# uthree/tinyvc

Measured on AMD Instinct MI355X. Metric: audio-samples/sec (16 kHz) end-to-end VC, higher is better.
Workload: dtype f32 (fp32 in / out / accumulate; channel contractions as two-term fp16 splits on v_mfma_f32_32x32x16_f16: 22-bit significands, three part-products per fp32 product)

## Files before the change

### tinyvc_amd/csrc/encoder.hip

```cpp
#include "conv3s.h"
#include "gemm_s2.h"
#include "cnx_s3.h"
#include "small_kernels.h"
#include "tvc_common.h"

namespace tvc {

constexpr int ENC_MTB = 4, ENC_NWV = 4, ENC_BPC = 2;

template <bool DW, int CPT>
static __global__ __launch_bounds__(1024) void dwconv_ln_kernel(const float* x, float* y,
                                                               const float* __restrict__ dw_w, const float* __restrict__ dw_b,
                                                               const float* __restrict__ g, const float* __restrict__ bta,
                                                               int C, int T, int dil, RagDev rg) {
    constexpr int NW = 16;
    const int rs = T;
    long ubase = (long)blockIdx.y * C * T;
    if (rg.tb) {
        T = rg.tb[blockIdx.y];
        ubase = rg.pre[blockIdx.y];
        if ((int)blockIdx.x * 64 >= T) return;
    }
    __shared__ float red[NW][64];
    constexpr bool STAGE = CPT >= 16;
    __shared__ __attribute__((aligned(16))) float Wl[STAGE ? 16 * CPT * 8 : 8];
    __shared__ float Gl[2][STAGE ? 16 * CPT : 1];
    if (STAGE) {
        for (int i = threadIdx.x; i < C; i += 1024) {
            if (DW) {
#pragma unroll
                for (int j = 0; j < 7; ++j) Wl[i * 8 + j] = dw_w[i * 7 + j];
                Wl[i * 8 + 7] = dw_b[i];
            }
            Gl[0][i] = g[i];
            Gl[1][i] = bta[i];
        }
        __syncthreads();
    }
    const int lane = threadIdx.x & 63, wave = threadIdx.x >> 6;
    const int t = blockIdx.x * 64 + lane;
    const bool ok = t < T;
    const int tc = ok ? t : T - 1;
    const float* xb = x + ubase;
    float* yb = y + ubase;

    int tt[7];
#pragma unroll
    for (int j = 0; j < 7; ++j) {
        int q = tc + (j - 3) * dil;
        tt[j] = q < 0 ? 0 : (q >= T ? T - 1 : q);
    }
    float v[CPT];
    float sum = 0.f;
#pragma unroll
    for (int i = 0; i < CPT; ++i) {
        const int c = wave + i * NW;
        if (DW) {
            const float* xr = xb + (long)c * rs;
            float wj[7], a;
            if (STAGE) {
                const float4 w0 = *reinterpret_cast<const float4*>(Wl + c * 8), w1 = *reinterpret_cast<const float4*>(Wl + c * 8 + 4);
                wj[0] = w0.x; wj[1] = w0.y; wj[2] = w0.z; wj[3] = w0.w; wj[4] = w1.x; wj[5] = w1.y; wj[6] = w1.z;
                a = w1.w;
            } else {
#pragma unroll
                for (int j = 0; j < 7; ++j) wj[j] = dw_w[c * 7 + j];
                a = dw_b[c];
            }
#pragma unroll
            for (int j = 0; j < 7; ++j) a = fmaf(wj[j], xr[tt[j]], a);
            v[i] = a;
        } else {
            v[i] = xb[(long)c * rs + tc];
        }
        sum += v[i];
    }
    red[wave][lane] = sum;
    __syncthreads();
    float tot = 0.f;
#pragma unroll
    for (int w = 0; w < NW; ++w) tot += red[w][lane];
    const float mean = tot / (float)C;
    __syncthreads();
    float sq = 0.f;
#pragma unroll
    for (int i = 0; i < CPT; ++i) {
        const float d = v[i] - mean;
        sq = fmaf(d, d, sq);
    }
    red[wave][lane] = sq;
    __syncthreads();
    float tot2 = 0.f;
#pragma unroll
    for (int w = 0; w < NW; ++w) tot2 += red[w][lane];
    const float var = tot2 / (float)C;
    const float rstd = 1.f / sqrtf(var + 1e-5f);
    if (!ok) return;
#pragma unroll
    for (int i = 0; i < CPT; ++i) {
        const int c = wave + i * NW;
        yb[(long)c * rs + t] = fmaf((v[i] - mean) * rstd, STAGE ? Gl[0][c] : g[c], STAGE ? Gl[1][c] : bta[c]);
    }
}
template <bool DW>
static int dwconv_ln_launch(tvc_ctx* ctx, hipStream_t s, const float* x, float* y, const float* dw_w, const float* dw_b, const float* g,
                            const float* bta, int B, int C, int T, int dil) {
    RagDev rg;
    TVC_CHECK(rag_view(ctx, s, 1, 0, &rg, nullptr));
    const dim3 grid(((ctx->rag ? ctx->rag->Tlong : T) + 63) / 64, ctx->rag ? ctx->rag->B : B), blk(1024);
    if (C == 384) hipLaunchKernelGGL((dwconv_ln_kernel<DW, 24>), grid, blk, 0, s, x, y, dw_w, dw_b, g, bta, C, T, dil, rg);
    else if (C == 128) hipLaunchKernelGGL((dwconv_ln_kernel<DW, 8>), grid, blk, 0, s, x, y, dw_w, dw_b, g, bta, C, T, dil, rg);
    else return fail(ctx, TVC_ERR_ARG, "dwconv_ln: unsupported channel count %d", C);
    return 0;
}

static __global__ void grn_norm_kernel(const float* __restrict__ h, float* __restrict__ gx, long rows, int T, RagDev rg, int C2) {
    const int lane = threadIdx.x & 63;
    long wave = (blockIdx.x * (long)blockDim.x + threadIdx.x) >> 6;
    long nwaves = ((long)gridDim.x * blockDim.x) >> 6;
    for (long r = wave; r < rows; r += nwaves) {
        const float* p = h + r * T;
        int n = T;
        if (rg.tb) {
            const int b = (int)(r / C2), c = (int)(r - (long)b * C2);
            p = h + (long)c * T + rg.pre[b];
            n = rg.tb[b];
        }
        float s = 0.f;
        for (int t = lane; t < n; t += 64) s = fmaf(p[t], p[t], s);
#pragma unroll
        for (int o = 32; o > 0; o >>= 1) s += __shfl_xor(s, o);
        if (lane == 0) gx[r] = sqrtf(s);
    }
}

static __global__ __launch_bounds__(256) void grn_finalize_kernel(const float* __restrict__ gx, const float* __restrict__ gamma,
                                                                  float* __restrict__ nx, int C2, float* __restrict__ hmax) {
    __shared__ float red[4];
    __shared__ float redm[4];
    const int b = blockIdx.x;
    const float* g = gx + (long)b * C2;
    float s = 0.f;
    for (int c = threadIdx.x; c < C2; c += 256) s += g[c];
#pragma unroll
    for (int o = 32; o > 0; o >>= 1) s += __shfl_xor(s, o);
    if ((threadIdx.x & 63) == 0) red[threadIdx.x >> 6] = s;
    __syncthreads();
    const float mean = (red[0] + red[1] + red[2] + red[3]) / (float)C2;
    const float den = mean + 1e-6f;
    float mx = 0.f;
    for (int c = threadIdx.x; c < C2; c += 256) {
        const float f = fmaf(gamma[c], g[c] / den, 1.f);
        nx[(long)b * C2 + c] = f;
        mx = fmaxf(mx, g[c] * fabsf(f));
    }
#pragma unroll
    for (int o = 32; o > 0; o >>= 1) mx = fmaxf(mx, __shfl_xor(mx, o));
    if ((threadIdx.x & 63) == 0) redm[threadIdx.x >> 6] = mx;
    __syncthreads();
    if (threadIdx.x == 0) hmax[b] = fmaxf(fmaxf(redm[0], redm[1]), fmaxf(redm[2], redm[3]));
}

int run_layernorm(tvc_ctx* ctx, hipStream_t s, float* x, const float* g, const float* b, int B, int C, int T) {
    TVC_CHECK(dwconv_ln_launch<false>(ctx, s, x, x, nullptr, nullptr, g, b, B, C, T, 1));
    return launch_check(ctx, "layernorm");
}

static __global__ void grn_tiles_kernel(float* __restrict__ gp, int gp_tiles, int K, int T, RagDev rg) {
    const int b = blockIdx.y, c = blockIdx.x * blockDim.x + threadIdx.x;
    if (c >= K) return;
    const int Tb = rg.tb ? rg.tb[b] : T, n = (Tb + 63) / 64;
    float* g = gp + (long)b * gp_tiles * K + c;
    float s = g[0];
    for (int t = 1; t < n; ++t) s += g[(long)t * K];
    g[0] = s;
}

template <int C>
static bool cnx_try(int* rc, tvc_ctx* ctx, hipStream_t s, const ConvNeXtW& w, float* x, float* h, float* gx, int B, int T, float* amax_out) {
    if (w.C != C || !(w.ln_bound < 32768.f) || w.c2.MT6 != 2 * C / 32 || w.c3.MT6 != C / 32 || w.c2.S6 < C / 16 || w.c3.S6 < 2 * C / 16) return false;
    const int NB = ctx->rag ? ctx->rag->B : B, Tl = ctx->rag ? ctx->rag->Tlong : T, rs = T;
    if ((long)rs * 8 * 4 >= (1L << 31)) return false;
    constexpr int KP = C == 384 ? 2 : 1;
    if ((*rc = lds_optin<cnx1_kernel<C, 1>>(ctx, Cnx1<C, 1>::LDS_BYTES, "cnx")) ||
        (*rc = lds_optin<cnx1_kernel<C, 2>>(ctx, Cnx1<C, 2>::LDS_BYTES, "cnx")) ||
        (*rc = lds_optin<cnx2_kernel<C, KP>>(ctx, Cnx2<C, KP>::LDS_BYTES, "cnx")))
        return true;
    CnxArgs a{};
    a.x = x;
    a.h = h;
    a.T = T;
    a.rs = rs;
    if ((*rc = rag_view(ctx, s, 1, 0, &a.rg, nullptr)) != 0) return true;
    auto split = [&](int MT, int tiles) {
        int d = 1;
        for (int c = 1; c <= MT; ++c)
            if (MT % c == 0 && (long)tiles * c <= ctx->ncu) d = c;
        return d;
    };
    {
        a.A6 = reinterpret_cast<const uint4*>(w.c2.A6);
        a.wsc = w.c2.wscale;
        a.bias = w.c2.bias;
        a.MT = w.c2.MT6;
        a.dw_w = w.dw_w;
        a.dw_b = w.dw_b;
        a.ln_g = w.ln_g;
        a.ln_b = w.ln_b;
        a.dil = w.dilation;
        const int nt = Tl <= 32 ? 1 : 2, tx = (Tl + 32 * nt - 1) / (32 * nt);
        a.gp = gx;
        a.gp_tiles = tx;
        const int d = split(a.MT, tx * NB);
        a.mt_per_wg = a.MT / d;
        const dim3 grid((unsigned)tx, (unsigned)NB, (unsigned)d);
        constexpr int nthr = Cnx1<C, 2>::NTHR, lds1 = Cnx1<C, 1>::LDS_BYTES, lds2 = Cnx1<C, 2>::LDS_BYTES;
        if (nt == 1) hipLaunchKernelGGL((cnx1_kernel<C, 1>), grid, dim3(nthr), lds1, s, a);
        else hipLaunchKernelGGL((cnx1_kernel<C, 2>), grid, dim3(nthr), lds2, s, a);
    }
    a.gp_sum = a.gp_tiles > CNX_GP_INLINE;
    if (a.gp_sum) hipLaunchKernelGGL(grn_tiles_kernel, dim3((2 * C + 255) / 256, (unsigned)NB), dim3(256), 0, s, gx, a.gp_tiles, 2 * C, T, a.rg);
    {
        a.A6 = reinterpret_cast<const uint4*>(w.c3.A6);
        a.wsc = w.c3.wscale;
        a.bias = w.c3_bias_grn;
        a.MT = w.c3.MT6;
        a.grn_g = w.grn_g;
        a.amax_y = amax_out;
        const int tx = (Tl + 63) / 64;
        const int d = split(a.MT, tx * NB);
        a.mt_per_wg = a.MT / d;
        constexpr int nthr = Cnx2<C, KP>::NTHR, lds = Cnx2<C, KP>::LDS_BYTES;
        hipLaunchKernelGGL((cnx2_kernel<C, KP>), dim3((unsigned)tx, (unsigned)NB, (unsigned)d), dim3(nthr), lds, s, a);
    }
    *rc = launch_check(ctx, "convnext (fused)");
    return true;
}

int run_convnext(tvc_ctx* ctx, hipStream_t s, Ws& ws, const ConvNeXtW& w, float* x, int B, int T, float* amax_out) {
    const int C = w.C, C2 = 2 * w.C, ncols = B * T;
    const int NB = ctx->rag ? ctx->rag->B : B;
    size_t mk = ws.mark();
    float* y = ws.get<float>((size_t)B * C * T);
    float* h = ws.get<float>((size_t)B * C2 * T);
    const int Tlong = ctx->rag ? ctx->rag->Tlong : T;
    float* gx = ws.get<float>((size_t)NB * C2 * ((Tlong + 63) / 64));
    float* nx = ws.get<float>((size_t)NB * C2);
    float* ymax = ws.get<float>((size_t)NB);
    float* hmax = ws.get<float>((size_t)NB);
    ws.release(mk);
    if (ws.dry) return 0;
    {
        int rc = 0;
        if (C == 384 ? cnx_try<384>(&rc, ctx, s, w, x, h, gx, B, T, amax_out) : (C == 128 && cnx_try<128>(&rc, ctx, s, w, x, h, gx, B, T, amax_out))) return rc;
    }
    {
        TVC_CHECK(dwconv_ln_launch<true>(ctx, s, x, y, w.dw_w, w.dw_b, w.ln_g, w.ln_b, B, C, T, w.dilation));
    }
    {
        const float* ym = nullptr;
        if (!(w.ln_bound < 32768.f)) {
            TVC_HIP(ctx, hipMemsetAsync(ymax, 0, (size_t)NB * sizeof(float), s));
            TVC_CHECK(run_amax_rows(ctx, s, y, B, C, T, ymax));
            ym = ymax;
        }
        EpiBias<ACT_GELU, false> ep{h, w.c2.bias, nullptr, C2, T, ncols, (long)C2 * T, 0};
        int rc = 0;
        if (!gemm_s2_try(&rc, ctx, s, w.c2, y, B, C, T, 0, ep, ym)) rc = gemm_s_launch<ENC_MTB, ENC_NWV, ENC_BPC>(ctx, s, w.c2, y, B, C, T, 0, ep, ym);
        TVC_CHECK(rc);
    }
    {
        RagDev rg;
        TVC_CHECK(rag_view(ctx, s, 1, 0, &rg, nullptr));
        hipLaunchKernelGGL(grn_norm_kernel, dim3(grid_for((long)NB * C2 * 64)), dim3(256), 0, s, h, gx, (long)NB * C2, T, rg, C2);
        hipLaunchKernelGGL(grn_finalize_kernel, dim3(NB), dim3(256), 0, s, gx, w.grn_g, nx, C2, hmax);
    }
    {
        EpiBias<ACT_NONE, true> ep{x, w.c3_bias_grn, x, C, T, ncols, (long)C * T, (long)C * T};
        int rc = 0;
        if (!gemm_s2_try<EpiBias<ACT_NONE, true>, true>(&rc, ctx, s, w.c3, h, B, C2, T, 0, ep, hmax, nx))
            rc = gemm_s_launch<ENC_MTB, ENC_NWV, ENC_BPC, EpiBias<ACT_NONE, true>, true>(ctx, s, w.c3, h, B, C2, T, 0, ep, hmax, nx);
        TVC_CHECK(rc);
    }
    if (amax_out) TVC_CHECK(run_amax_rows(ctx, s, x, B, C, T, amax_out));
    return launch_check(ctx, "convnext");
}

struct EpiSplit {
    static constexpr bool kIgemm = true;
    float* y0;
    float* y1;
    const float* bias;
    int M0, M1, T, ncols;
    __device__ __forceinline__ void store(int n, int m, const float v[4]) const {
        if (n >= ncols) return;
        int b = n / T, t = n - b * T;
#pragma unroll
        for (int r = 0; r < 4; ++r) {
            int mm = m + r;
            float o = v[r] + bias[mm < M0 + M1 ? mm : 0];
            if (mm < M0)
                y0[((long)b * M0 + mm) * T + t] = o;
            else if (mm < M0 + M1)
                y1[((long)b * M1 + mm - M0) * T + t] = o;
        }
    }
};

struct PTop4 {
    float v[4];
    int i[4];
    __device__ __forceinline__ void init() {
#pragma unroll
        for (int j = 0; j < 4; ++j) { v[j] = -INFINITY; i[j] = 0x7fffffff; }
    }
    __device__ __forceinline__ static bool better(float a, int ia, float b, int ib) { return a > b || (a == b && ia < ib); }
    __device__ __forceinline__ void insert(float x, int ix) {
        if (!better(x, ix, v[3], i[3])) return;
        if (better(x, ix, v[0], i[0])) { v[3] = v[2]; i[3] = i[2]; v[2] = v[1]; i[2] = i[1]; v[1] = v[0]; i[1] = i[0]; v[0] = x; i[0] = ix; }
        else if (better(x, ix, v[1], i[1])) { v[3] = v[2]; i[3] = i[2]; v[2] = v[1]; i[2] = i[1]; v[1] = x; i[1] = ix; }
        else if (better(x, ix, v[2], i[2])) { v[3] = v[2]; i[3] = i[2]; v[2] = x; i[2] = ix; }
        else { v[3] = x; i[3] = ix; }
    }
};

constexpr int kPdWaves = 16;
static __global__ __launch_bounds__(kPdWaves * 64) void pitch_decode_kernel(const float* __restrict__ logits, const float* __restrict__ freq,
                                                                  float* __restrict__ f0, int B, int T, float* __restrict__ f0s, float shift,
                                                                  const float* __restrict__ shifts, const int* __restrict__ col2b) {
    __shared__ float sv[kPdWaves][4][64];
    __shared__ int si[kPdWaves][4][64];
    const int lane = threadIdx.x & 63, wave = threadIdx.x >> 6;
    const long ncols = (long)B * T;
    const long n = blockIdx.x * 64L + lane;
    const bool ok = n < ncols;
    const long nn = ok ? n : ncols - 1;
    const int b = (int)(nn / T), t = (int)(nn - (long)b * T);
    const float* p = logits + (long)b * kPitchClasses * T + t;
    PTop4 top;
    top.init();
    constexpr int CPW = kPitchClasses / kPdWaves;
    float xv[CPW];
#pragma unroll
    for (int j = 0; j < CPW; ++j) xv[j] = p[(long)(wave * CPW + j) * T];
#pragma unroll
    for (int j = 0; j < CPW; ++j) {
        const float x = xv[j];
        top.insert(x != x ? INFINITY : x, wave * CPW + j);
    }
#pragma unroll
    for (int e = 0; e < 4; ++e) { sv[wave][e][lane] = top.v[e]; si[wave][e][lane] = top.i[e]; }
    __syncthreads();
    if (wave != 0 || !ok) return;
    for (int w = 1; w < kPdWaves; ++w)
#pragma unroll
        for (int e = 0; e < 4; ++e) top.insert(sv[w][e][lane], si[w][e][lane]);
#pragma unroll
    for (int e = 0; e < 4; ++e) top.i[e] = (unsigned)top.i[e] < (unsigned)kPitchClasses ? top.i[e] : 0;
    const float v0 = top.v[0];
    float e0 = 1.f, e1 = (float)exp((double)(top.v[1] - v0)), e2 = (float)exp((double)(top.v[2] - v0)), e3 = (float)exp((double)(top.v[3] - v0));
    float den = ((e0 + e1) + e2) + e3;
    float acc = __fmul_rn(e0 / den, freq[top.i[0]]);
    acc = __fadd_rn(acc, __fmul_rn(e1 / den, freq[top.i[1]]));
    acc = __fadd_rn(acc, __fmul_rn(e2 / den, freq[top.i[2]]));
    acc = __fadd_rn(acc, __fmul_rn(e3 / den, freq[top.i[3]]));
    const float fv = acc <= 20.f ? 0.f : acc;
    f0[n] = fv;
    if (f0s) f0s[n] = shift_frequency_one(fv, shifts ? shifts[col2b ? col2b[n] : b] : shift);
}

int run_pitch_decode(tvc_ctx* ctx, hipStream_t s, const float* logits, float* f0, int B, int T) {
    if (!ctx->pitch_freq) return fail(ctx, TVC_ERR_STATE, "pitch table not uploaded (tvc_set_pitch_table + tvc_finalize_weights)");
    const long ncols = (long)B * T;
    hipLaunchKernelGGL(pitch_decode_kernel, dim3((unsigned)((ncols + 63) / 64)), dim3(kPdWaves * 64), 0, s, logits, ctx->pitch_freq, f0, B, T, (float*)nullptr, 0.f, (const float*)nullptr, (const int*)nullptr);
    return launch_check(ctx, "pitch_decode");
}

int run_encoder(tvc_ctx* ctx, hipStream_t s, Ws& ws, const float* spec, float* ssl, float* f0,
                float* logits, int B, int T, const float* spec_bound, float* zeroed_slots, float* f0_shifted, float shift, const float* shifts) {
    const int ncols = B * T;
    float* xs = ws.get<float>((size_t)B * kSslCh * T);
    float* xp = ws.get<float>((size_t)B * kPitchCh * T);
    float* lg = logits ? logits : ws.get<float>((size_t)B * kPitchClasses * T);
    const int NB = ctx->rag ? ctx->rag->B : B;
    float* slots = zeroed_slots ? zeroed_slots : ws.get<float>((size_t)3 * NB);
    float *spec_max = slots, *xs_max = slots + NB, *xp_max = slots + 2 * NB;
    if (!ws.dry) {
        if (!zeroed_slots) TVC_HIP(ctx, hipMemsetAsync(slots, 0, (size_t)3 * NB * sizeof(float), s));
        if (spec_bound) spec_max = const_cast<float*>(spec_bound);
        else TVC_CHECK(run_amax_rows(ctx, s, spec, B, kBins, T, spec_max));
        EpiSplit ep{xs, xp, ctx->enc_in.bias, kSslCh, kPitchCh, T, ncols};
        TVC_CHECK((gemm_s_launch_ragged<ENC_MTB, ENC_NWV, ENC_BPC>(ctx, s, ctx->enc_in, spec, B, kBins, T, (long)kBins * T, ep, spec_max)));
        TVC_CHECK(run_layernorm(ctx, s, xs, ctx->ssl_ln_g, ctx->ssl_ln_b, B, kSslCh, T));
        TVC_CHECK(run_layernorm(ctx, s, xp, ctx->pit_ln_g, ctx->pit_ln_b, B, kPitchCh, T));
    }
    const int gtiles = ((ctx->rag ? ctx->rag->Tlong : T) + 63) / 64;
    const size_t ssl_scratch = ((size_t)B * kSslCh * T * 3 + (size_t)NB * kSslCh * 2 * (gtiles + 1)) * sizeof(float) + (size_t)NB * 8 + 4096;
    char* ssl_blk = ws.get<char>(ssl_scratch);
    Ws wssl(ssl_blk, ssl_scratch, ws.dry);
    SideFork fk(ctx, s);
    TVC_CHECK(fk.fork(ws, ctx->ev_fork, ctx->ev_join));
    const hipStream_t sp = fk.side;
    for (int i = 0; i < 4; ++i) TVC_CHECK(run_convnext(ctx, sp, ws, ctx->pit_mid[i], xp, B, T, i == 3 ? xp_max : nullptr));
    if (!ws.dry) {
        EpiBias<ACT_NONE, false> ep{lg, ctx->pit_out.bias, nullptr, kPitchClasses, T, ncols, (long)kPitchClasses * T, 0};
        int rc = 0;
        if (!gemm_s2_try(&rc, ctx, sp, ctx->pit_out, xp, B, kPitchCh, T, 0, ep, xp_max)) rc = gemm_s_launch<ENC_MTB, ENC_NWV, ENC_BPC>(ctx, sp, ctx->pit_out, xp, B, kPitchCh, T, 0, ep, xp_max);
        TVC_CHECK(rc);
        hipLaunchKernelGGL(pitch_decode_kernel, dim3((ncols + 63) / 64), dim3(kPdWaves * 64), 0, sp, lg, ctx->pitch_freq, f0, B, T, f0_shifted, shift, shifts,
                           shifts && ctx->rag ? ctx->rag->d_col2b : (const int*)nullptr);
    }
    TVC_CHECK(fk.end());
    for (int i = 0; i < 6; ++i) TVC_CHECK(run_convnext(ctx, s, wssl, ctx->ssl_mid[i], xs, B, T, i == 5 ? xs_max : nullptr));
    if (wssl.peak > wssl.cap) return fail(ctx, TVC_ERR_WORKSPACE, "encoder: SSL scratch block too small");
    if (ws.dry) return 0;
    {
        EpiBias<ACT_NONE, false> ep{ssl, ctx->ssl_out.bias, nullptr, kSslDim, T, ncols, (long)kSslDim * T, 0};
        int rc = 0;
        if (!gemm_s2_try(&rc, ctx, s, ctx->ssl_out, xs, B, kSslCh, T, 0, ep, xs_max)) rc = gemm_s_launch<ENC_MTB, ENC_NWV, ENC_BPC>(ctx, s, ctx->ssl_out, xs, B, kSslCh, T, 0, ep, xs_max);
        TVC_CHECK(rc);
    }
    TVC_CHECK(fk.join());
    return launch_check(ctx, "encoder");
}

int run_ssl_amax(tvc_ctx* ctx, hipStream_t s, const float* ssl, int B, int T, float* slot) { return run_amax_rows(ctx, s, ssl, B, kSslDim, T, slot); }

}
```

### tinyvc_amd/csrc/gemm_s2.h

```cpp
#pragma once
#include "gemm_epi.h"
#include "split_fp16.h"

namespace tvc {

constexpr int G2_NWV_MIN = 2;

struct Gemm2Args {
    const uint4* A6;
    const float* wsc;
    const float* amax_x;
    int MT;
    const float* x;
    unsigned xstride;
    int Cin, T, ncols;
    const float* kscale;
    int ncoltiles, mblocks, vtiles;
    const int* col2b;
};

template <int NWV_, int WN_>
struct G2Tile {
    static constexpr int NWV = NWV_, WN = WN_, MTB = 4, WM = 2;
    static constexpr int NW = 2 * NWV, NTHR = NW * 64, BM = 128, BN = NWV * WN * 32;
    static constexpr int A_U4 = 2 * MTB * kPU4;
    static constexpr int X_U4 = 2 * kParts * 2 * BN;
    static constexpr int BUF_U4 = A_U4 + X_U4;
    static constexpr int X_PER = WN;
    static constexpr int A_PIECES = 2 * MTB * kParts, A_PER = (A_PIECES + NW - 1) / NW;
    static constexpr int lds_bytes = 2 * BUF_U4 * 16;
};

template <int NWV, int WN, class Epi, bool SCALED>
__global__ __launch_bounds__(2 * NWV * 64) void gemm_s2_kernel(Gemm2Args a, Epi ep) {
    using TL = G2Tile<NWV, WN>;
    constexpr int BN = TL::BN, NW = TL::NW, A_PER = TL::A_PER, X_PER = TL::X_PER;
    extern __shared__ __attribute__((aligned(16))) uint4 smem_g2[];
    const int tid = threadIdx.x, lane = tid & 63;
    const int wave = __builtin_amdgcn_readfirstlane(tid >> 6);
    const int l31 = lane & 31, lh = lane >> 5;
    const int wm = wave / NWV, wn = wave - wm * NWV;
    const int nslab = a.Cin / 32;
    const int stride = gridDim.x;

    auto coords = [&](int v, int& mt0, int& n0) __attribute__((always_inline)) -> bool {
        const int r = v & 7, u = v >> 3;
        const int mb = u % a.mblocks;
        const int nt = (u / a.mblocks) * 8 + r;
        mt0 = mb * TL::MTB;
        n0 = nt * BN;
        return nt < a.ncoltiles;
    };
    auto next_valid = [&](int v) __attribute__((always_inline)) -> int {
        int m_, n_;
        while (v < a.vtiles && !coords(v, m_, n_)) v += stride;
        return v;
    };

    u32x4 ar[A_PER];
    float xr[X_PER][8];
    u32x4 kr[X_PER][2];
    unsigned xo[X_PER], ko[X_PER];
    float xsc[X_PER];
    int xdst[X_PER];
#pragma unroll
    for (int i = 0; i < X_PER; ++i) {
        const int idx = tid + i * TL::NTHR;
        const int gk = idx / BN, c = idx - gk * BN;
        xdst[i] = (gk >> 1) * (2 * kParts * BN) + (gk & 1) * BN + c;
    }
    auto tile_offsets = [&](int n0) __attribute__((always_inline)) {
#pragma unroll
        for (int i = 0; i < X_PER; ++i) {
            const int idx = tid + i * TL::NTHR;
            const int gk = idx / BN, c = idx - gk * BN;
            int p = n0 + c;
            p = p < a.ncols ? p : a.ncols - 1;
            const int b = p / a.T, t = p - b * a.T;
            const int bu = a.col2b ? a.col2b[p] : b;
            xo[i] = (unsigned)b * a.xstride + (unsigned)(gk * 8 * a.T + t);
            ko[i] = (unsigned)(bu * a.Cin + gk * 8);
            xsc[i] = bfp_load(a.amax_x, bu).s;
        }
    };
    int lv = next_valid(blockIdx.x), ls = 0, lmt0 = 0, ln0 = 0;
    if (lv >= a.vtiles) return;
    coords(lv, lmt0, ln0);
    int cv = lv, cs = 0, cmt0 = lmt0, cn0 = ln0;
    tile_offsets(ln0);

    auto issue_load = [&]() __attribute__((always_inline)) {
        const uint4* abase = a.A6 + ((long)ls * 2 * a.MT + lmt0) * kPU4;
#pragma unroll
        for (int i = 0; i < A_PER; ++i) {
            int q = wave + i * NW;
            q = q < TL::A_PIECES ? q : TL::A_PIECES - 1;
            const int kg = q / (TL::MTB * kParts), rem = q - kg * (TL::MTB * kParts);
            ar[i] = ldg_so4(abase, 16u * (unsigned)(kg * a.MT * kPU4 + rem * 64 + lane));
        }
        const float* xc = a.x + (long)ls * 32 * a.T;
#pragma unroll
        for (int i = 0; i < X_PER; ++i)
#pragma unroll
            for (int j = 0; j < 8; ++j) xr[i][j] = ldg_so(xc + (long)j * a.T, 4u * xo[i]);
        if constexpr (SCALED) {
            const uint4* kc = reinterpret_cast<const uint4*>(a.kscale + ls * 32);
#pragma unroll
            for (int i = 0; i < X_PER; ++i) {
                kr[i][0] = ldg_so4(kc, 4u * ko[i]);
                kr[i][1] = ldg_so4(kc, 4u * ko[i] + 16u);
            }
        }
    };
    auto advance_load = [&]() __attribute__((always_inline)) {
        if (++ls == nslab) {
            const int v2 = next_valid(lv + stride);
            if (v2 < a.vtiles) {
                lv = v2;
                ls = 0;
                coords(lv, lmt0, ln0);
                tile_offsets(ln0);
            } else {
                ls = nslab - 1;
            }
        }
    };
    auto lstore = [&](int buf) __attribute__((always_inline)) {
        uint4* Ab = smem_g2 + buf * TL::BUF_U4;
        uint4* Xb = Ab + TL::A_U4;
#pragma unroll
        for (int i = 0; i < A_PER; ++i) {
            int q = wave + i * NW;
            q = q < TL::A_PIECES ? q : TL::A_PIECES - 1;
            *reinterpret_cast<u32x4*>(Ab + q * 64 + lane) = ar[i];
        }
#pragma unroll
        for (int i = 0; i < X_PER; ++i) {
            if constexpr (SCALED) {
                typedef float f32x4 __attribute__((ext_vector_type(4)));
                const f32x4 k0 = __builtin_bit_cast(f32x4, kr[i][0]), k1 = __builtin_bit_cast(f32x4, kr[i][1]);
                xr[i][0] *= k0.x; xr[i][1] *= k0.y; xr[i][2] *= k0.z; xr[i][3] *= k0.w;
                xr[i][4] *= k1.x; xr[i][5] *= k1.y; xr[i][6] *= k1.z; xr[i][7] *= k1.w;
            }
#pragma unroll
            for (int j = 0; j < 8; ++j) xr[i][j] *= xsc[i];
            uint4 p1, p2;
            split8(xr[i], p1, p2);
            Xb[xdst[i]] = p1;
            Xb[2 * BN + xdst[i]] = p2;
        }
    };

    f32x16 hi[2][WN], lo[2][WN];
#pragma unroll
    for (int i = 0; i < 2; ++i)
#pragma unroll
        for (int j = 0; j < WN; ++j)
#pragma unroll
            for (int r = 0; r < 16; ++r) hi[i][j][r] = lo[i][j][r] = 0.f;
    auto multiply = [&](int buf, int kg) __attribute__((always_inline)) {
        const uint4* Ab = smem_g2 + buf * TL::BUF_U4 + (kg * TL::MTB * kParts + wm * 2 * kParts) * 64 + lane;
        const uint4* Xb = smem_g2 + buf * TL::BUF_U4 + TL::A_U4 + kg * (2 * kParts * BN) + lh * BN + wn * WN * 32 + l31;
        f16x8 af[2][kParts], bf[WN][kParts];
#pragma unroll
        for (int j = 0; j < WN; ++j)
#pragma unroll
            for (int p = 0; p < kParts; ++p) bf[j][p] = __builtin_bit_cast(f16x8, Xb[p * 2 * BN + j * 32]);
#pragma unroll
        for (int i = 0; i < 2; ++i)
#pragma unroll
            for (int p = 0; p < kParts; ++p) af[i][p] = __builtin_bit_cast(f16x8, Ab[(i * kParts + p) * 64]);
#pragma unroll
        for (int i = 0; i < 2; ++i)
#pragma unroll
            for (int j = 0; j < WN; ++j) lo[i][j] = TVC_MFMA16(af[i][1], bf[j][0], lo[i][j]);
#pragma unroll
        for (int i = 0; i < 2; ++i)
#pragma unroll
            for (int j = 0; j < WN; ++j) hi[i][j] = TVC_MFMA16(af[i][0], bf[j][0], hi[i][j]);
#pragma unroll
        for (int i = 0; i < 2; ++i)
#pragma unroll
            for (int j = 0; j < WN; ++j) lo[i][j] = TVC_MFMA16(af[i][0], bf[j][1], lo[i][j]);
    };

    issue_load();
    advance_load();
    lstore(0);
    issue_load();
    advance_load();
    slab_barrier();
    int buf = 0;
    while (true) {
        multiply(buf, 0);
        lstore(buf ^ 1);
        issue_load();
        multiply(buf, 1);
        advance_load();
        if (++cs == nslab) {
#pragma unroll
            for (int i = 0; i < 2; ++i) {
                const float cw = a.wsc[cmt0 + wm * 2 + i];
#pragma unroll
                for (int j = 0; j < WN; ++j) {
                    const int n = cn0 + (wn * WN + j) * 32 + l31;
                    const int nc = n < a.ncols ? n : a.ncols - 1;
                    const float c = cw * bfp_load(a.amax_x, a.col2b ? a.col2b[nc] : nc / a.T).inv, cl = c * kLoInv;
#pragma unroll
                    for (int q = 0; q < 4; ++q) {
                        const float v[4] = {comb(hi[i][j][4 * q], lo[i][j][4 * q], c, cl), comb(hi[i][j][4 * q + 1], lo[i][j][4 * q + 1], c, cl),
                                            comb(hi[i][j][4 * q + 2], lo[i][j][4 * q + 2], c, cl), comb(hi[i][j][4 * q + 3], lo[i][j][4 * q + 3], c, cl)};
                        ep.store(n, (cmt0 + wm * 2 + i) * 32 + 8 * q + 4 * lh, v);
                    }
#pragma unroll
                    for (int r = 0; r < 16; ++r) hi[i][j][r] = lo[i][j][r] = 0.f;
                }
            }
            cs = 0;
            cv = next_valid(cv + stride);
            if (cv >= a.vtiles) break;
            coords(cv, cmt0, cn0);
        }
        slab_barrier();
        buf ^= 1;
    }
}

template <int NWV, int WN, class Epi, bool SCALED>
inline int gemm_s2_launch_t(tvc_ctx* ctx, hipStream_t s, const PackedW& w, const float* x, int B, int Cin, int T, long xstride, const Epi& ep,
                            const float* kscale, const float* amax_x) {
    using TL = G2Tile<NWV, WN>;
    TVC_CHECK((lds_optin<gemm_s2_kernel<NWV, WN, Epi, SCALED>>(ctx, TL::lds_bytes, "gemm_s2")));
    Gemm2Args a;
    a.A6 = reinterpret_cast<const uint4*>(w.A6);
    a.wsc = w.wscale;
    a.amax_x = amax_x;
    a.MT = w.MT6;
    a.x = x;
    a.xstride = (unsigned)(xstride ? xstride : (long)Cin * T);
    a.Cin = Cin;
    a.T = T;
    a.ncols = B * T;
    a.kscale = kscale;
    a.mblocks = w.MT6 / TL::MTB;
    a.ncoltiles = (a.ncols + TL::BN - 1) / TL::BN;
    a.vtiles = (a.ncoltiles + 7) / 8 * 8 * a.mblocks;
    a.col2b = nullptr;
    if (ctx->rag) {
        if (B != 1 || T != ctx->rag->Ttot) return fail(ctx, TVC_ERR_STATE, "gemm_s2: a ragged batch runs as one long utterance at the frame rate");
        a.col2b = ctx->rag->d_col2b;
    }
    const int slots = ctx->ncu / 8 * 8;
    dim3 g((unsigned)(a.vtiles < slots ? a.vtiles : slots));
    hipLaunchKernelGGL((gemm_s2_kernel<NWV, WN, Epi, SCALED>), g, dim3(TL::NTHR), TL::lds_bytes, s, a, ep);
    return 0;
}

template <class Epi, bool SCALED = false>
inline bool gemm_s2_try(int* rc, tvc_ctx* ctx, hipStream_t s, const PackedW& w, const float* x, int B, int Cin, int T, long xstride, const Epi& ep,
                        const float* amax_x, const float* kscale = nullptr) {
    const long xs = xstride ? xstride : (long)Cin * T;
    if (Cin % 32 != 0 || Cin / 16 > w.S6 || w.MT6 % 4 != 0 || xs * B >= (1L << 29) || (long)B * T >= (1L << 29) || (SCALED && !kscale)) return false;
    const long ncols = (long)B * T;
    const int mblocks = w.MT6 / 4, slots = ctx->ncu / 8 * 8;
    int best = 4;
    long best_cost = -1;
    for (int nwv = G2_NWV_MIN; nwv <= 6; ++nwv) {
        const long tiles = (ncols + nwv * 32 - 1) / (nwv * 32) * mblocks;
        const long rounds = (tiles + slots - 1) / slots;
        const long cost = rounds * (nwv * 32 + 64);
        if (best_cost < 0 || cost < best_cost) { best_cost = cost; best = nwv; }
    }
    if (best == 2) *rc = gemm_s2_launch_t<2, 1, Epi, SCALED>(ctx, s, w, x, B, Cin, T, xstride, ep, kscale, amax_x);
    else if (best == 3) *rc = gemm_s2_launch_t<3, 1, Epi, SCALED>(ctx, s, w, x, B, Cin, T, xstride, ep, kscale, amax_x);
    else if (best == 4) *rc = gemm_s2_launch_t<4, 1, Epi, SCALED>(ctx, s, w, x, B, Cin, T, xstride, ep, kscale, amax_x);
    else if (best == 5) *rc = gemm_s2_launch_t<5, 1, Epi, SCALED>(ctx, s, w, x, B, Cin, T, xstride, ep, kscale, amax_x);
    else *rc = gemm_s2_launch_t<6, 1, Epi, SCALED>(ctx, s, w, x, B, Cin, T, xstride, ep, kscale, amax_x);
    return true;
}

}
```

Measured before the change: 691.5 million.

## Route encoder input projection through gemm_s2 with K-tail clamping and deeper prefetch ring

Adds a CLAMP variant of the gemm_s2 kernel that handles an input channel count that is not a multiple of 32 by clamping row loads. This lets the encoder's spectrogram input projection use gemm_s2 instead of the older gemm_s ragged path. It also adds a templated register ring depth D, set to 2 for unscaled NWV=4, so global loads are prefetched two slabs ahead, and restructures the slab loop into an unrolled macro step. The deeper ring costs registers and may reduce occupancy, and clamped rows rely on zero-padded packed weights for the K tail.

```diff
diff --git a/tinyvc_amd/csrc/encoder.hip b/tinyvc_amd/csrc/encoder.hip
--- a/tinyvc_amd/csrc/encoder.hip
+++ b/tinyvc_amd/csrc/encoder.hip
@@ -390,7 +390,10 @@
         if (spec_bound) spec_max = const_cast<float*>(spec_bound);
         else TVC_CHECK(run_amax_rows(ctx, s, spec, B, kBins, T, spec_max));
         EpiSplit ep{xs, xp, ctx->enc_in.bias, kSslCh, kPitchCh, T, ncols};
-        TVC_CHECK((gemm_s_launch_ragged<ENC_MTB, ENC_NWV, ENC_BPC>(ctx, s, ctx->enc_in, spec, B, kBins, T, (long)kBins * T, ep, spec_max)));
+        int rc = 0;
+        if (!gemm_s2_try_ktail(&rc, ctx, s, ctx->enc_in, spec, B, kBins, T, (long)kBins * T, ep, spec_max))
+            rc = gemm_s_launch_ragged<ENC_MTB, ENC_NWV, ENC_BPC>(ctx, s, ctx->enc_in, spec, B, kBins, T, (long)kBins * T, ep, spec_max);
+        TVC_CHECK(rc);
         TVC_CHECK(run_layernorm(ctx, s, xs, ctx->ssl_ln_g, ctx->ssl_ln_b, B, kSslCh, T));
         TVC_CHECK(run_layernorm(ctx, s, xp, ctx->pit_ln_g, ctx->pit_ln_b, B, kPitchCh, T));
     }
diff --git a/tinyvc_amd/csrc/gemm_s2.h b/tinyvc_amd/csrc/gemm_s2.h
--- a/tinyvc_amd/csrc/gemm_s2.h
+++ b/tinyvc_amd/csrc/gemm_s2.h
@@ -16,6 +16,7 @@
     int Cin, T, ncols;
     const float* kscale;
     int ncoltiles, mblocks, vtiles;
+    int kmax;
     const int* col2b;
 };
 
@@ -31,7 +32,10 @@
     static constexpr int lds_bytes = 2 * BUF_U4 * 16;
 };
 
-template <int NWV, int WN, class Epi, bool SCALED>
+template <int NWV, bool SCALED>
+constexpr int g2_depth() { return !SCALED && NWV == 4 ? 2 : 1; }
+
+template <int NWV, int WN, class Epi, bool SCALED, bool CLAMP, int D>
 __global__ __launch_bounds__(2 * NWV * 64) void gemm_s2_kernel(Gemm2Args a, Epi ep) {
     using TL = G2Tile<NWV, WN>;
     constexpr int BN = TL::BN, NW = TL::NW, A_PER = TL::A_PER, X_PER = TL::X_PER;
@@ -57,9 +61,10 @@
         return v;
     };
 
-    u32x4 ar[A_PER];
-    float xr[X_PER][8];
-    u32x4 kr[X_PER][2];
+    u32x4 ar[D][A_PER];
+    float xr[D][X_PER][8];
+    u32x4 kr[D][X_PER][2];
+    float xscr[D][X_PER];
     unsigned xo[X_PER], ko[X_PER];
     float xsc[X_PER];
     int xdst[X_PER];
@@ -69,6 +74,10 @@
         const int gk = idx / BN, c = idx - gk * BN;
         xdst[i] = (gk >> 1) * (2 * kParts * BN) + (gk & 1) * BN + c;
     }
+    auto col_bfp = [&](int p, int b) __attribute__((always_inline)) -> Bfp {
+        if (!a.amax_x) return Bfp{1.f, 1.f};
+        return bfp_from_amax(a.amax_x[a.col2b ? a.col2b[p] : b]);
+    };
     auto tile_offsets = [&](int n0) __attribute__((always_inline)) {
 #pragma unroll
         for (int i = 0; i < X_PER; ++i) {
@@ -77,10 +86,15 @@
             int p = n0 + c;
             p = p < a.ncols ? p : a.ncols - 1;
             const int b = p / a.T, t = p - b * a.T;
-            const int bu = a.col2b ? a.col2b[p] : b;
-            xo[i] = (unsigned)b * a.xstride + (unsigned)(gk * 8 * a.T + t);
-            ko[i] = (unsigned)(bu * a.Cin + gk * 8);
-            xsc[i] = bfp_load(a.amax_x, bu).s;
+            xo[i] = (unsigned)b * a.xstride + (unsigned)((CLAMP ? 0 : gk * 8 * a.T) + t);
+            if constexpr (SCALED) {
+                const int bu = a.col2b ? a.col2b[p] : b;
+                ko[i] = (unsigned)(bu * a.Cin + gk * 8);
+                xsc[i] = bfp_load(a.amax_x, bu).s;
+            } else {
+                ko[i] = 0;
+                xsc[i] = col_bfp(p, b).s;
+            }
         }
     };
     int lv = next_valid(blockIdx.x), ls = 0, lmt0 = 0, ln0 = 0;
@@ -89,26 +103,40 @@
     int cv = lv, cs = 0, cmt0 = lmt0, cn0 = ln0;
     tile_offsets(ln0);
 
-    auto issue_load = [&]() __attribute__((always_inline)) {
+    auto issue_load = [&](int r) __attribute__((always_inline)) {
         const uint4* abase = a.A6 + ((long)ls * 2 * a.MT + lmt0) * kPU4;
 #pragma unroll
         for (int i = 0; i < A_PER; ++i) {
             int q = wave + i * NW;
             q = q < TL::A_PIECES ? q : TL::A_PIECES - 1;
             const int kg = q / (TL::MTB * kParts), rem = q - kg * (TL::MTB * kParts);
-            ar[i] = ldg_so4(abase, 16u * (unsigned)(kg * a.MT * kPU4 + rem * 64 + lane));
-        }
-        const float* xc = a.x + (long)ls * 32 * a.T;
-#pragma unroll
-        for (int i = 0; i < X_PER; ++i)
-#pragma unroll
-            for (int j = 0; j < 8; ++j) xr[i][j] = ldg_so(xc + (long)j * a.T, 4u * xo[i]);
+            ar[r][i] = ldg_so4(abase, 16u * (unsigned)(kg * a.MT * kPU4 + rem * 64 + lane));
+        }
+        if constexpr (CLAMP) {
+#pragma unroll
+            for (int i = 0; i < X_PER; ++i) {
+                const int row0 = ls * 32 + (tid + i * TL::NTHR) / BN * 8;
+#pragma unroll
+                for (int j = 0; j < 8; ++j) {
+                    const int row = row0 + j < a.kmax ? row0 + j : a.kmax;
+                    xr[r][i][j] = ldg_so(a.x, 4u * (xo[i] + (unsigned)(row * a.T)));
+                }
+            }
+        } else {
+            const float* xc = a.x + (long)ls * 32 * a.T;
+#pragma unroll
+            for (int i = 0; i < X_PER; ++i)
+#pragma unroll
+                for (int j = 0; j < 8; ++j) xr[r][i][j] = ldg_so(xc + (long)j * a.T, 4u * xo[i]);
+        }
+#pragma unroll
+        for (int i = 0; i < X_PER; ++i) xscr[r][i] = xsc[i];
         if constexpr (SCALED) {
             const uint4* kc = reinterpret_cast<const uint4*>(a.kscale + ls * 32);
 #pragma unroll
             for (int i = 0; i < X_PER; ++i) {
-                kr[i][0] = ldg_so4(kc, 4u * ko[i]);
-                kr[i][1] = ldg_so4(kc, 4u * ko[i] + 16u);
+                kr[r][i][0] = ldg_so4(kc, 4u * ko[i]);
+                kr[r][i][1] = ldg_so4(kc, 4u * ko[i] + 16u);
             }
         }
     };
@@ -125,27 +153,27 @@
             }
         }
     };
-    auto lstore = [&](int buf) __attribute__((always_inline)) {
+    auto lstore = [&](int buf, int r) __attribute__((always_inline)) {
         uint4* Ab = smem_g2 + buf * TL::BUF_U4;
         uint4* Xb = Ab + TL::A_U4;
 #pragma unroll
         for (int i = 0; i < A_PER; ++i) {
             int q = wave + i * NW;
             q = q < TL::A_PIECES ? q : TL::A_PIECES - 1;
-            *reinterpret_cast<u32x4*>(Ab + q * 64 + lane) = ar[i];
+            *reinterpret_cast<u32x4*>(Ab + q * 64 + lane) = ar[r][i];
         }
 #pragma unroll
         for (int i = 0; i < X_PER; ++i) {
             if constexpr (SCALED) {
                 typedef float f32x4 __attribute__((ext_vector_type(4)));
-                const f32x4 k0 = __builtin_bit_cast(f32x4, kr[i][0]), k1 = __builtin_bit_cast(f32x4, kr[i][1]);
-                xr[i][0] *= k0.x; xr[i][1] *= k0.y; xr[i][2] *= k0.z; xr[i][3] *= k0.w;
-                xr[i][4] *= k1.x; xr[i][5] *= k1.y; xr[i][6] *= k1.z; xr[i][7] *= k1.w;
-            }
-#pragma unroll
-            for (int j = 0; j < 8; ++j) xr[i][j] *= xsc[i];
+                const f32x4 k0 = __builtin_bit_cast(f32x4, kr[r][i][0]), k1 = __builtin_bit_cast(f32x4, kr[r][i][1]);
+                xr[r][i][0] *= k0.x; xr[r][i][1] *= k0.y; xr[r][i][2] *= k0.z; xr[r][i][3] *= k0.w;
+                xr[r][i][4] *= k1.x; xr[r][i][5] *= k1.y; xr[r][i][6] *= k1.z; xr[r][i][7] *= k1.w;
+            }
+#pragma unroll
+            for (int j = 0; j < 8; ++j) xr[r][i][j] *= xscr[r][i];
             uint4 p1, p2;
-            split8(xr[i], p1, p2);
+            split8(xr[r][i], p1, p2);
             Xb[xdst[i]] = p1;
             Xb[2 * BN + xdst[i]] = p2;
         }
@@ -184,53 +212,70 @@
             for (int j = 0; j < WN; ++j) lo[i][j] = TVC_MFMA16(af[i][0], bf[j][1], lo[i][j]);
     };
 
-    issue_load();
-    advance_load();
-    lstore(0);
-    issue_load();
+    int buf = 0;
+    auto slab = [&](int r) __attribute__((always_inline)) {
+        multiply(buf, 0);
+        lstore(buf ^ 1, r);
+        issue_load(r);
+        multiply(buf, 1);
+        advance_load();
+    };
+    bool done = false;
+    auto tile_end = [&]() __attribute__((always_inline)) {
+#pragma unroll
+        for (int i = 0; i < 2; ++i) {
+            const float cw = a.wsc[cmt0 + wm * 2 + i];
+#pragma unroll
+            for (int j = 0; j < WN; ++j) {
+                const int n = cn0 + (wn * WN + j) * 32 + l31;
+                const int nc = n < a.ncols ? n : a.ncols - 1;
+                const float c = cw * col_bfp(nc, nc / a.T).inv, cl = c * kLoInv;
+#pragma unroll
+                for (int q = 0; q < 4; ++q) {
+                    const float v[4] = {comb(hi[i][j][4 * q], lo[i][j][4 * q], c, cl), comb(hi[i][j][4 * q + 1], lo[i][j][4 * q + 1], c, cl),
+                                        comb(hi[i][j][4 * q + 2], lo[i][j][4 * q + 2], c, cl), comb(hi[i][j][4 * q + 3], lo[i][j][4 * q + 3], c, cl)};
+                    ep.store(n, (cmt0 + wm * 2 + i) * 32 + 8 * q + 4 * lh, v);
+                }
+#pragma unroll
+                for (int e = 0; e < 16; ++e) hi[i][j][e] = lo[i][j][e] = 0.f;
+            }
+        }
+        cs = 0;
+        cv = next_valid(cv + stride);
+        if (cv >= a.vtiles) done = true;
+        else coords(cv, cmt0, cn0);
+    };
+
+#pragma unroll
+    for (int r = 0; r < D; ++r) {
+        issue_load(r);
+        advance_load();
+    }
+    lstore(0, 0);
+    issue_load(0);
     advance_load();
     slab_barrier();
-    int buf = 0;
-    while (true) {
-        multiply(buf, 0);
-        lstore(buf ^ 1);
-        issue_load();
-        multiply(buf, 1);
-        advance_load();
-        if (++cs == nslab) {
-#pragma unroll
-            for (int i = 0; i < 2; ++i) {
-                const float cw = a.wsc[cmt0 + wm * 2 + i];
-#pragma unroll
-                for (int j = 0; j < WN; ++j) {
-                    const int n = cn0 + (wn * WN + j) * 32 + l31;
-                    const int nc = n < a.ncols ? n : a.ncols - 1;
-                    const float c = cw * bfp_load(a.amax_x, a.col2b ? a.col2b[nc] : nc / a.T).inv, cl = c * kLoInv;
-#pragma unroll
-                    for (int q = 0; q < 4; ++q) {
-                        const float v[4] = {comb(hi[i][j][4 * q], lo[i][j][4 * q], c, cl), comb(hi[i][j][4 * q + 1], lo[i][j][4 * q + 1], c, cl),
-                                            comb(hi[i][j][4 * q + 2], lo[i][j][4 * q + 2], c, cl), comb(hi[i][j][4 * q + 3], lo[i][j][4 * q + 3], c, cl)};
-                        ep.store(n, (cmt0 + wm * 2 + i) * 32 + 8 * q + 4 * lh, v);
-                    }
-#pragma unroll
-                    for (int r = 0; r < 16; ++r) hi[i][j][r] = lo[i][j][r] = 0.f;
-                }
-            }
-            cs = 0;
-            cv = next_valid(cv + stride);
-            if (cv >= a.vtiles) break;
-            coords(cv, cmt0, cn0);
-        }
-        slab_barrier();
-        buf ^= 1;
-    }
-}
-
-template <int NWV, int WN, class Epi, bool SCALED>
+    static_assert(D >= 1 && D <= 4, "the slab loop is written out for up to four ring sets");
+#define TVC_G2_STEP(r)                                                                       \
+    slab(r);                                                                                 \
+    if (++cs == nslab && !done) tile_end();                                                  \
+    slab_barrier();  \
+    buf ^= 1;
+    do {
+        TVC_G2_STEP(1 % D)
+        if constexpr (D > 1) { TVC_G2_STEP(2 % D) }
+        if constexpr (D > 2) { TVC_G2_STEP(3 % D) }
+        if constexpr (D > 3) { TVC_G2_STEP(0) }
+    } while (!done);
+#undef TVC_G2_STEP
+}
+
+template <int NWV, int WN, class Epi, bool SCALED, bool CLAMP>
 inline int gemm_s2_launch_t(tvc_ctx* ctx, hipStream_t s, const PackedW& w, const float* x, int B, int Cin, int T, long xstride, const Epi& ep,
-                            const float* kscale, const float* amax_x) {
+                            const float* kscale, const float* amax_x, int krows) {
     using TL = G2Tile<NWV, WN>;
-    TVC_CHECK((lds_optin<gemm_s2_kernel<NWV, WN, Epi, SCALED>>(ctx, TL::lds_bytes, "gemm_s2")));
+    constexpr int D = g2_depth<NWV, SCALED>();
+    TVC_CHECK((lds_optin<gemm_s2_kernel<NWV, WN, Epi, SCALED, CLAMP, D>>(ctx, TL::lds_bytes, "gemm_s2")));
     Gemm2Args a;
     a.A6 = reinterpret_cast<const uint4*>(w.A6);
     a.wsc = w.wscale;
@@ -239,6 +284,7 @@
     a.x = x;
     a.xstride = (unsigned)(xstride ? xstride : (long)Cin * T);
     a.Cin = Cin;
+    a.kmax = krows - 1;
     a.T = T;
     a.ncols = B * T;
     a.kscale = kscale;
@@ -252,13 +298,13 @@
     }
     const int slots = ctx->ncu / 8 * 8;
     dim3 g((unsigned)(a.vtiles < slots ? a.vtiles : slots));
-    hipLaunchKernelGGL((gemm_s2_kernel<NWV, WN, Epi, SCALED>), g, dim3(TL::NTHR), TL::lds_bytes, s, a, ep);
+    hipLaunchKernelGGL((gemm_s2_kernel<NWV, WN, Epi, SCALED, CLAMP, D>), g, dim3(TL::NTHR), TL::lds_bytes, s, a, ep);
     return 0;
 }
 
-template <class Epi, bool SCALED = false>
-inline bool gemm_s2_try(int* rc, tvc_ctx* ctx, hipStream_t s, const PackedW& w, const float* x, int B, int Cin, int T, long xstride, const Epi& ep,
-                        const float* amax_x, const float* kscale = nullptr) {
+template <class Epi, bool SCALED, bool CLAMP>
+inline bool gemm_s2_dispatch(int* rc, tvc_ctx* ctx, hipStream_t s, const PackedW& w, const float* x, int B, int Cin, int krows, int T, long xstride, const Epi& ep,
+                             const float* amax_x, const float* kscale) {
     const long xs = xstride ? xstride : (long)Cin * T;
     if (Cin % 32 != 0 || Cin / 16 > w.S6 || w.MT6 % 4 != 0 || xs * B >= (1L << 29) || (long)B * T >= (1L << 29) || (SCALED && !kscale)) return false;
     const long ncols = (long)B * T;
@@ -271,12 +317,23 @@
         const long cost = rounds * (nwv * 32 + 64);
         if (best_cost < 0 || cost < best_cost) { best_cost = cost; best = nwv; }
     }
-    if (best == 2) *rc = gemm_s2_launch_t<2, 1, Epi, SCALED>(ctx, s, w, x, B, Cin, T, xstride, ep, kscale, amax_x);
-    else if (best == 3) *rc = gemm_s2_launch_t<3, 1, Epi, SCALED>(ctx, s, w, x, B, Cin, T, xstride, ep, kscale, amax_x);
-    else if (best == 4) *rc = gemm_s2_launch_t<4, 1, Epi, SCALED>(ctx, s, w, x, B, Cin, T, xstride, ep, kscale, amax_x);
-    else if (best == 5) *rc = gemm_s2_launch_t<5, 1, Epi, SCALED>(ctx, s, w, x, B, Cin, T, xstride, ep, kscale, amax_x);
-    else *rc = gemm_s2_launch_t<6, 1, Epi, SCALED>(ctx, s, w, x, B, Cin, T, xstride, ep, kscale, amax_x);
+    if (best == 2) *rc = gemm_s2_launch_t<2, 1, Epi, SCALED, CLAMP>(ctx, s, w, x, B, Cin, T, xstride, ep, kscale, amax_x, krows);
+    else if (best == 3) *rc = gemm_s2_launch_t<3, 1, Epi, SCALED, CLAMP>(ctx, s, w, x, B, Cin, T, xstride, ep, kscale, amax_x, krows);
+    else if (best == 4) *rc = gemm_s2_launch_t<4, 1, Epi, SCALED, CLAMP>(ctx, s, w, x, B, Cin, T, xstride, ep, kscale, amax_x, krows);
+    else if (best == 5) *rc = gemm_s2_launch_t<5, 1, Epi, SCALED, CLAMP>(ctx, s, w, x, B, Cin, T, xstride, ep, kscale, amax_x, krows);
+    else *rc = gemm_s2_launch_t<6, 1, Epi, SCALED, CLAMP>(ctx, s, w, x, B, Cin, T, xstride, ep, kscale, amax_x, krows);
     return true;
 }
-
-}
+template <class Epi, bool SCALED = false>
+inline bool gemm_s2_try(int* rc, tvc_ctx* ctx, hipStream_t s, const PackedW& w, const float* x, int B, int Cin, int T, long xstride, const Epi& ep,
+                        const float* amax_x, const float* kscale = nullptr) {
+    return gemm_s2_dispatch<Epi, SCALED, false>(rc, ctx, s, w, x, B, Cin, Cin, T, xstride, ep, amax_x, kscale);
+}
+template <class Epi>
+inline bool gemm_s2_try_ktail(int* rc, tvc_ctx* ctx, hipStream_t s, const PackedW& w, const float* x, int B, int krows, int T, long xstride, const Epi& ep,
+                              const float* amax_x) {
+    if (krows < 1 || xstride < (long)krows * T) return false;
+    return gemm_s2_dispatch<Epi, false, true>(rc, ctx, s, w, x, B, (krows + 31) / 32 * 32, krows, T, xstride, ep, amax_x, nullptr);
+}
+
+}
```

Result: no change. 690.3 million (-0.2%).
